# Hanbo-Cheng/DAWN-pytorch

Measured on NVIDIA H100. Metric: denoising-steps/sec (200-frame 256^2 clip), higher is better.
Workload: dtype f32

## Files before the change

### dawn_pytorch_b200/csrc/tc_common.cuh

```cuda
#pragma once
#include <cuda_fp16.h>
#include <type_traits>
#include "common.cuh"

namespace dawn {
namespace tc {

__device__ __forceinline__ uint32_t smem_u32(const void* p) { return (uint32_t)__cvta_generic_to_shared(p); }

__device__ __forceinline__ uint8_t* smem_align1024(uint8_t* base) { return base + ((1024u - (smem_u32(base) & 1023u)) & 1023u); }

template <uint32_t R>
__device__ __forceinline__ void setmaxnreg_dec() { asm volatile("setmaxnreg.dec.sync.aligned.u32 %0;" ::"n"(R)); }
template <uint32_t R>
__device__ __forceinline__ void setmaxnreg_inc() { asm volatile("setmaxnreg.inc.sync.aligned.u32 %0;" ::"n"(R)); }

template <int I, int N, class F>
__device__ __forceinline__ void static_for(F&& f) {
  if constexpr (I < N) {
    f(std::integral_constant<int, I>{});
    static_for<I + 1, N>(f);
  }
}

__device__ __forceinline__ void mbar_init(uint64_t* bar, uint32_t count) {
  asm volatile("mbarrier.init.shared::cta.b64 [%0], %1;" ::"r"(smem_u32(bar)), "r"(count));
}
__device__ __forceinline__ void mbar_arrive(uint64_t* bar) {
  asm volatile("mbarrier.arrive.shared::cta.b64 _, [%0];" ::"r"(smem_u32(bar)) : "memory");
}
__device__ __forceinline__ void mbar_arrive_relaxed(uint64_t* bar) {
  asm volatile("mbarrier.arrive.relaxed.cta.shared::cta.b64 _, [%0];" ::"r"(smem_u32(bar)) : "memory");
}
__device__ __forceinline__ void mbar_arrive_expect_tx(uint64_t* bar, uint32_t bytes) {
  asm volatile("mbarrier.arrive.expect_tx.shared::cta.b64 _, [%0], %1;" ::"r"(smem_u32(bar)), "r"(bytes) : "memory");
}
__device__ __forceinline__ void mbar_wait(uint64_t* bar, uint32_t parity) {
  asm volatile(
      "{\n\t"
      ".reg .pred p;\n\t"
      "WAIT_LOOP:\n\t"
      "mbarrier.try_wait.parity.shared::cta.b64 p, [%0], %1;\n\t"
      "@p bra WAIT_DONE;\n\t"
      "bra WAIT_LOOP;\n\t"
      "WAIT_DONE:\n\t"
      "}" ::"r"(smem_u32(bar)), "r"(parity)
      : "memory");
}
__device__ __forceinline__ void bulk_copy_g2s(void* smem_dst, const void* gsrc, uint32_t bytes, uint64_t* bar) {
  asm volatile("cp.async.bulk.shared::cluster.global.mbarrier::complete_tx::bytes [%0], [%1], %2, [%3];" ::"r"(smem_u32(smem_dst)),
               "l"(gsrc), "r"(bytes), "r"(smem_u32(bar))
               : "memory");
}
__device__ __forceinline__ void fence_proxy_async() { asm volatile("fence.proxy.async.shared::cta;" ::: "memory"); }

__device__ __forceinline__ void wgmma_fence() { asm volatile("wgmma.fence.sync.aligned;" ::: "memory"); }
__device__ __forceinline__ void wgmma_commit() { asm volatile("wgmma.commit_group.sync.aligned;" ::: "memory"); }
template <int N>
__device__ __forceinline__ void wgmma_wait() { asm volatile("wgmma.wait_group.sync.aligned %0;" ::"n"(N) : "memory"); }
__device__ __forceinline__ void wgmma_fence_acc(float (&d)[32]) {
#pragma unroll
  for (int i = 0; i < 32; ++i) asm volatile("" : "+f"(d[i])::"memory");
}
__device__ __forceinline__ void wgmma_m64n64k16(float (&d)[32], uint64_t adesc, uint64_t bdesc, uint32_t scale_d) {
  asm volatile(
      "{\n\t"
      ".reg .pred p;\n\t"
      "setp.ne.b32 p, %34, 0;\n\t"
      "wgmma.mma_async.sync.aligned.m64n64k16.f32.f16.f16 "
      "{%0, %1, %2, %3, %4, %5, %6, %7, %8, %9, %10, %11, %12, %13, %14, %15, "
      "%16, %17, %18, %19, %20, %21, %22, %23, %24, %25, %26, %27, %28, %29, %30, %31}, %32, %33, p, 1, 1, 0, 0;\n\t"
      "}"
      : "+f"(d[0]), "+f"(d[1]), "+f"(d[2]), "+f"(d[3]), "+f"(d[4]), "+f"(d[5]), "+f"(d[6]), "+f"(d[7]), "+f"(d[8]), "+f"(d[9]),
        "+f"(d[10]), "+f"(d[11]), "+f"(d[12]), "+f"(d[13]), "+f"(d[14]), "+f"(d[15]), "+f"(d[16]), "+f"(d[17]), "+f"(d[18]),
        "+f"(d[19]), "+f"(d[20]), "+f"(d[21]), "+f"(d[22]), "+f"(d[23]), "+f"(d[24]), "+f"(d[25]), "+f"(d[26]), "+f"(d[27]),
        "+f"(d[28]), "+f"(d[29]), "+f"(d[30]), "+f"(d[31])
      : "l"(adesc), "l"(bdesc), "r"(scale_d)
      : "memory");
}

__device__ __forceinline__ uint64_t make_desc(uint32_t saddr, uint32_t sbo = 1024) {
  return (uint64_t)((saddr >> 4) & 0x3FFF) | (1ull << 16) | ((uint64_t)((sbo >> 4) & 0x3FFF) << 32) | (1ull << 62);
}

constexpr int kStageLd = 68;
__device__ __forceinline__ void stage_fragment(float* stage, int r0, const float (&d)[32], bool first, int wtid) {
  const int w = wtid >> 5, l = wtid & 31;
  float* p0 = stage + (size_t)(r0 + w * 16 + (l >> 2)) * kStageLd + 2 * (l & 3);
  float* p1 = p0 + 8 * kStageLd;
#pragma unroll
  for (int j = 0; j < 8; ++j) {
    float2* a = reinterpret_cast<float2*>(p0 + 8 * j);
    float2* b = reinterpret_cast<float2*>(p1 + 8 * j);
    if (first) {
      *a = make_float2(d[4 * j], d[4 * j + 1]);
      *b = make_float2(d[4 * j + 2], d[4 * j + 3]);
    } else {
      const float2 x = *a, y = *b;
      *a = make_float2(x.x + d[4 * j], x.y + d[4 * j + 1]);
      *b = make_float2(y.x + d[4 * j + 2], y.y + d[4 * j + 3]);
    }
  }
}

__device__ __forceinline__ uint32_t swz(int r, int c) { return (uint32_t)((r >> 3) * 1024 + (r & 7) * 128 + ((c ^ (r & 7)) << 4)); }

__device__ __forceinline__ void split_f16x2(float x0, float x1, uint32_t& hi, uint32_t& lo) {
  const float h0 = __uint_as_float((__float_as_uint(x0) + 0x1000u) & 0xFFFFE000u);
  const float h1 = __uint_as_float((__float_as_uint(x1) + 0x1000u) & 0xFFFFE000u);
  const __half2 h = __floats2half2_rn(h0, h1);
  const __half2 l = __floats2half2_rn(x0 - h0, x1 - h1);
  hi = *reinterpret_cast<const uint32_t*>(&h);
  lo = *reinterpret_cast<const uint32_t*>(&l);
}

__device__ __forceinline__ void store_rows_coalesced(float* wbuf, const float (&acc)[64], float* out, size_t opix, int ldo,
                                                     int n0, bool rv, int lane) {
  float* dst[4];
#pragma unroll
  for (int k = 0; k < 4; ++k) {
    const int r = (lane >> 2) + 8 * k;
    const uint32_t lo = __shfl_sync(0xffffffffu, (uint32_t)opix, r);
    const uint32_t hi = __shfl_sync(0xffffffffu, (uint32_t)((unsigned long long)opix >> 32), r);
    const int ok = __shfl_sync(0xffffffffu, rv ? 1 : 0, r);
    const size_t px = ((size_t)hi << 32) | lo;
    dst[k] = ok ? (out + px * ldo + n0 + (lane & 3) * 4) : nullptr;
  }
#pragma unroll
  for (int pass = 0; pass < 4; ++pass) {
    __syncwarp();
#pragma unroll
    for (int j = 0; j < 4; ++j)
      *reinterpret_cast<float4*>(wbuf + lane * 20 + j * 4) =
          make_float4(acc[pass * 16 + j * 4], acc[pass * 16 + j * 4 + 1], acc[pass * 16 + j * 4 + 2], acc[pass * 16 + j * 4 + 3]);
    __syncwarp();
#pragma unroll
    for (int k = 0; k < 4; ++k) {
      const int r = (lane >> 2) + 8 * k;
      const float4 v = *reinterpret_cast<const float4*>(wbuf + r * 20 + (lane & 3) * 4);
      if (dst[k]) *reinterpret_cast<float4*>(dst[k] + pass * 16) = v;
    }
  }
}

}
}
```

### dawn_pytorch_b200/csrc/temporal_fused.cu

```cuda
#include <cuda_fp16.h>
#include <cmath>
#include <cstring>
#include <vector>
#include <algorithm>
#include "common.cuh"
#include "kernels.cuh"
#include "temporal_fused.cuh"

namespace dawn {
namespace {

constexpr int C = 64;
constexpr int X_LD = C + 8;
constexpr int W_LD = C + 8;
constexpr int K_LD = 40;
constexpr int WO_LD = 40;
constexpr int NTH = 512;
constexpr int NWARP = NTH / 32;
constexpr int W_STAGE = 2 * 96 * W_LD + 2 * 64 * WO_LD;
constexpr float LOG2E = 1.4426950408889634f;

__device__ __forceinline__ void mma16816(float (&d)[4], const uint32_t (&a)[4], uint32_t b0, uint32_t b1) {
  asm volatile(
      "mma.sync.aligned.m16n8k16.row.col.f32.f16.f16.f32 {%0,%1,%2,%3}, {%4,%5,%6,%7}, {%8,%9}, {%0,%1,%2,%3};\n"
      : "+f"(d[0]), "+f"(d[1]), "+f"(d[2]), "+f"(d[3])
      : "r"(a[0]), "r"(a[1]), "r"(a[2]), "r"(a[3]), "r"(b0), "r"(b1));
}
__device__ __forceinline__ void ldsm4(uint32_t (&r)[4], const __half* p) {
  const uint32_t addr = (uint32_t)__cvta_generic_to_shared(p);
  asm volatile("ldmatrix.sync.aligned.m8n8.x4.shared.b16 {%0,%1,%2,%3}, [%4];\n"
               : "=r"(r[0]), "=r"(r[1]), "=r"(r[2]), "=r"(r[3]) : "r"(addr));
}
__device__ __forceinline__ void ldsm4_trans(uint32_t (&r)[4], const __half* p) {
  const uint32_t addr = (uint32_t)__cvta_generic_to_shared(p);
  asm volatile("ldmatrix.sync.aligned.m8n8.x4.trans.shared.b16 {%0,%1,%2,%3}, [%4];\n"
               : "=r"(r[0]), "=r"(r[1]), "=r"(r[2]), "=r"(r[3]) : "r"(addr));
}
__device__ __forceinline__ void cp_async_16(void* dst, const void* src) {
  const uint32_t d = (uint32_t)__cvta_generic_to_shared(dst);
  asm volatile("cp.async.cg.shared.global [%0], [%1], 16;\n" :: "r"(d), "l"(src) : "memory");
}
__device__ __forceinline__ void cp_async_commit() { asm volatile("cp.async.commit_group;\n" ::: "memory"); }
__device__ __forceinline__ void cp_async_wait_all() { asm volatile("cp.async.wait_group 0;\n" ::: "memory"); }
__device__ __forceinline__ float ex2(float x) {
  float y;
  asm("ex2.approx.ftz.f32 %0, %1;\n" : "=f"(y) : "f"(x));
  return y;
}
__device__ __forceinline__ void split2h(float x0, float x1, uint32_t& hi, uint32_t& lo) {
  const float h0 = __uint_as_float(__float_as_uint(x0) & 0xFFFFE000u);
  const float h1 = __uint_as_float(__float_as_uint(x1) & 0xFFFFE000u);
  const __half2 h = __floats2half2_rn(h0, h1);
  const __half2 l = __floats2half2_rn(x0 - h0, x1 - h1);
  hi = *reinterpret_cast<const uint32_t*>(&h);
  lo = *reinterpret_cast<const uint32_t*>(&l);
}
__device__ __forceinline__ void mma3(float (&acc)[4], const uint32_t (&ah)[4], const uint32_t (&al)[4], const uint32_t (&b)[4]) {
  mma16816(acc, al, b[0], b[1]);
  mma16816(acc, ah, b[2], b[3]);
  mma16816(acc, ah, b[0], b[1]);
}

__global__ void __launch_bounds__(NTH, 1) temporal_fused_kernel(TemporalFusedArgs a) {
  extern __shared__ __align__(16) unsigned char tf_smem[];
  const int F = a.F;
  const int Fp = (F + 15) & ~15;
  const int KROWS = Fp + 32;
  const int nbuf = a.nbuf;
  __half* Xh = reinterpret_cast<__half*>(tf_smem);
  __half* Xl = Xh + Fp * X_LD;
  __half* Kh = Xl + Fp * X_LD;
  __half* Kl = Kh + KROWS * K_LD;
  __half* Vh = Kl + KROWS * K_LD;
  __half* Vl = Vh + KROWS * K_LD;
  __half* Wst = Vl + KROWS * K_LD;
  float* s_stat = reinterpret_cast<float*>(Wst + nbuf * W_STAGE);
  float* s_bias = s_stat + 2 * Fp;

  const int tid = threadIdx.x, warp = tid >> 5, lane = tid & 31;
  const int g = lane >> 2, t = lane & 3;
  const int lm = lane >> 3, lr = lane & 7;
  const int pix = blockIdx.x;
  const int band = a.band;
  const int nbias = 2 * band + 1;

  for (int i = tid; i < 8 * nbias; i += NTH) s_bias[i] = a.bias[i] * LOG2E;
  {
    const int l16 = tid & 15;
    for (int f0 = 0; f0 < Fp; f0 += NTH / 16) {
      const int f = f0 + (tid >> 4);
      float4 v = make_float4(0.f, 0.f, 0.f, 0.f);
      if (f < F) v = __ldg(reinterpret_cast<const float4*>(a.x + ((size_t)f * a.P + pix) * a.ldx) + l16);
      float s = (v.x + v.y) + (v.z + v.w);
#pragma unroll
      for (int o = 1; o < 16; o <<= 1) s += __shfl_xor_sync(0xffffffffu, s, o);
      const float mu = s * (1.0f / C);
      const float d0 = v.x - mu, d1 = v.y - mu, d2 = v.z - mu, d3 = v.w - mu;
      float ss = (d0 * d0 + d1 * d1) + (d2 * d2 + d3 * d3);
#pragma unroll
      for (int o = 1; o < 16; o <<= 1) ss += __shfl_xor_sync(0xffffffffu, ss, o);
      if (f < Fp) {
        if (l16 == 0) { s_stat[2 * f] = mu; s_stat[2 * f + 1] = 1.0f / sqrtf(ss * (1.0f / C) + 1e-5f); }
        uint32_t h0, l0, h1, l1;
        split2h(v.x, v.y, h0, l0); split2h(v.z, v.w, h1, l1);
        *reinterpret_cast<uint2*>(&Xh[f * X_LD + l16 * 4]) = make_uint2(h0, h1);
        *reinterpret_cast<uint2*>(&Xl[f * X_LD + l16 * 4]) = make_uint2(l0, l1);
      }
    }
    for (int i = tid; i < (KROWS - F) * K_LD; i += NTH) {
      Kh[F * K_LD + i] = __float2half(0.f); Kl[F * K_LD + i] = __float2half(0.f);
      Vh[F * K_LD + i] = __float2half(0.f); Vl[F * K_LD + i] = __float2half(0.f);
    }
  }

  const int ntiles = Fp >> 4;
  const int qtile = (a.q_lo >> 4) + warp;
  const bool has_q = qtile * 16 < a.q_hi;
  float y[8][4];
#pragma unroll
  for (int n = 0; n < 8; ++n)
#pragma unroll
    for (int c = 0; c < 4; ++c) y[n][c] = 0.f;

  int head_off = 0;
  const __half* Wh = Wst;
  auto stage_weights = [&](int head, __half* dst) {
    const uint4* src = reinterpret_cast<const uint4*>(a.Wqkv + (size_t)head * 2 * 96 * C);
    for (int i = tid; i < 2 * 96 * C / 8; i += NTH) {
      const int r = i / (C / 8), c8 = i - r * (C / 8);
      cp_async_16(dst + r * W_LD + c8 * 8, src + i);
    }
    const uint4* so = reinterpret_cast<const uint4*>(a.Wout + (size_t)head * 2 * 64 * 32);
    __half* od = dst + 2 * 96 * W_LD;
    for (int i = tid; i < 2 * 64 * 32 / 8; i += NTH) {
      const int r = i >> 2, c8 = i & 3;
      cp_async_16(od + r * WO_LD + c8 * 8, so + i);
    }
    cp_async_commit();
  };
  auto project = [&](int f0, int part, float (&acc)[4][4]) {
#pragma unroll
    for (int n = 0; n < 4; ++n)
#pragma unroll
      for (int c = 0; c < 4; ++c) acc[n][c] = 0.f;
#pragma unroll
    for (int ks = 0; ks < 4; ++ks) {
      uint32_t ah[4], al[4];
      const int aoff = (f0 + (lm & 1) * 8 + lr) * X_LD + ks * 16 + (lm >> 1) * 8;
      ldsm4(ah, Xh + aoff);
      ldsm4(al, Xl + aoff);
#pragma unroll
      for (int n = 0; n < 4; ++n) {
        uint32_t b[4];
        ldsm4(b, Wh + ((lm >> 1) * 96 + part * 32 + n * 8 + lr) * W_LD + ks * 16 + (lm & 1) * 8);
        mma3(acc[n], ah, al, b);
      }
    }
    const float mu0 = s_stat[2 * (f0 + g)], rs0 = s_stat[2 * (f0 + g) + 1];
    const float mu1 = s_stat[2 * (f0 + g + 8)], rs1 = s_stat[2 * (f0 + g + 8) + 1];
    const int fr0 = min(f0 + g, F - 1), fr1 = min(f0 + g + 8, F - 1);
#pragma unroll
    for (int n = 0; n < 4; ++n) {
      const float2 w = __ldg(reinterpret_cast<const float2*>(a.wsum + part * 256 + head_off + n * 8 + 2 * t));
      acc[n][0] = rs0 * (acc[n][0] * a.inv_wscale - mu0 * w.x);
      acc[n][1] = rs0 * (acc[n][1] * a.inv_wscale - mu0 * w.y);
      acc[n][2] = rs1 * (acc[n][2] * a.inv_wscale - mu1 * w.x);
      acc[n][3] = rs1 * (acc[n][3] * a.inv_wscale - mu1 * w.y);
      if (part < 2) {
        const float2 cs0 = __ldg(reinterpret_cast<const float2*>(a.rot) + (size_t)fr0 * 16 + n * 4 + t);
        const float2 cs1 = __ldg(reinterpret_cast<const float2*>(a.rot) + (size_t)fr1 * 16 + n * 4 + t);
        const float x0 = acc[n][0], x1 = acc[n][1], x2 = acc[n][2], x3 = acc[n][3];
        acc[n][0] = x0 * cs0.x - x1 * cs0.y; acc[n][1] = x1 * cs0.x + x0 * cs0.y;
        acc[n][2] = x2 * cs1.x - x3 * cs1.y; acc[n][3] = x3 * cs1.x + x2 * cs1.y;
      }
    }
  };

  if (nbuf == 2) stage_weights(0, Wst);
  for (int head = 0; head < 8; ++head) {
    if (nbuf == 2) {
      cp_async_wait_all();
      __syncthreads();
      Wh = Wst + (head & 1) * W_STAGE;
      if (head + 1 < 8) stage_weights(head + 1, Wst + ((head + 1) & 1) * W_STAGE);
    } else {
      __syncthreads();
      stage_weights(head, Wst);
      cp_async_wait_all();
      __syncthreads();
    }
    const __half* Oh = Wh + 2 * 96 * W_LD;
    head_off = head * 32;

    for (int tile = warp; tile < ntiles; tile += NWARP) {
      const int f0 = tile * 16, fr0 = f0 + g, fr1 = f0 + g + 8;
      float acc[4][4];
      project(f0, 1, acc);
#pragma unroll
      for (int n = 0; n < 4; ++n) {
        uint32_t h0, l0, h1, l1;
        split2h(acc[n][0], acc[n][1], h0, l0); split2h(acc[n][2], acc[n][3], h1, l1);
        *reinterpret_cast<uint32_t*>(&Kh[fr0 * K_LD + n * 8 + 2 * t]) = h0;
        *reinterpret_cast<uint32_t*>(&Kl[fr0 * K_LD + n * 8 + 2 * t]) = l0;
        *reinterpret_cast<uint32_t*>(&Kh[fr1 * K_LD + n * 8 + 2 * t]) = h1;
        *reinterpret_cast<uint32_t*>(&Kl[fr1 * K_LD + n * 8 + 2 * t]) = l1;
      }
      project(f0, 2, acc);
#pragma unroll
      for (int n = 0; n < 4; ++n) {
        uint32_t h0, l0, h1, l1;
        split2h(acc[n][0], acc[n][1], h0, l0); split2h(acc[n][2], acc[n][3], h1, l1);
        *reinterpret_cast<uint32_t*>(&Vh[fr0 * K_LD + n * 8 + 2 * t]) = h0;
        *reinterpret_cast<uint32_t*>(&Vl[fr0 * K_LD + n * 8 + 2 * t]) = l0;
        *reinterpret_cast<uint32_t*>(&Vh[fr1 * K_LD + n * 8 + 2 * t]) = h1;
        *reinterpret_cast<uint32_t*>(&Vl[fr1 * K_LD + n * 8 + 2 * t]) = l1;
      }
    }
    uint32_t qh[2][4], ql[2][4];
    if (has_q) {
      float acc[4][4];
      project(qtile * 16, 0, acc);
#pragma unroll
      for (int n = 0; n < 4; ++n)
#pragma unroll
        for (int c = 0; c < 4; ++c) acc[n][c] *= LOG2E;
#pragma unroll
      for (int ks = 0; ks < 2; ++ks) {
        split2h(acc[2 * ks][0], acc[2 * ks][1], qh[ks][0], ql[ks][0]);
        split2h(acc[2 * ks][2], acc[2 * ks][3], qh[ks][1], ql[ks][1]);
        split2h(acc[2 * ks + 1][0], acc[2 * ks + 1][1], qh[ks][2], ql[ks][2]);
        split2h(acc[2 * ks + 1][2], acc[2 * ks + 1][3], qh[ks][3], ql[ks][3]);
      }
    }
    __syncthreads();
    if (!has_q) continue;

    const float* bias = s_bias + head * nbias + band;
    const int i0 = qtile * 16;
    float o[4][4], mrow[2] = {-1e30f, -1e30f}, lrow[2] = {0.f, 0.f};
#pragma unroll
    for (int n = 0; n < 4; ++n)
#pragma unroll
      for (int c = 0; c < 4; ++c) o[n][c] = 0.f;
    const int kr_lo = max(0, i0 - band) & ~7, kr_hi = min(F, i0 + 16 + band);
    for (int kr0 = kr_lo; kr0 < kr_hi; kr0 += 32) {
      float s[4][4];
#pragma unroll
      for (int n = 0; n < 4; ++n)
#pragma unroll
        for (int c = 0; c < 4; ++c) s[n][c] = 0.f;
#pragma unroll
      for (int ks = 0; ks < 2; ++ks)
#pragma unroll
        for (int n = 0; n < 4; ++n) {
          uint32_t b[4];
          ldsm4(b, ((lm & 2) ? Kl : Kh) + (kr0 + n * 8 + lr) * K_LD + ks * 16 + (lm & 1) * 8);
          mma3(s[n], qh[ks], ql[ks], b);
        }
      float mnew[2] = {mrow[0], mrow[1]};
      const int rel0 = kr0 - i0 + 2 * t - g;
      const bool edge = (kr0 + 31 - i0 > band) || (kr0 - i0 - 15 < -band) || (kr0 + 32 > F);
      if (edge) {
#pragma unroll
        for (int n = 0; n < 4; ++n)
#pragma unroll
          for (int c = 0; c < 4; ++c) {
            const int rel = rel0 + n * 8 + (c & 1) - ((c & 2) ? 8 : 0);
            const bool v = ((unsigned)(rel + band) <= (unsigned)(2 * band)) && (kr0 + n * 8 + 2 * t + (c & 1) < F);
            s[n][c] = v ? s[n][c] + bias[v ? rel : 0] : -1e30f;
            mnew[c >> 1] = fmaxf(mnew[c >> 1], s[n][c]);
          }
      } else {
#pragma unroll
        for (int n = 0; n < 4; ++n)
#pragma unroll
          for (int c = 0; c < 4; ++c) {
            s[n][c] += bias[rel0 + n * 8 + (c & 1) - ((c & 2) ? 8 : 0)];
            mnew[c >> 1] = fmaxf(mnew[c >> 1], s[n][c]);
          }
      }
#pragma unroll
      for (int r = 0; r < 2; ++r) {
        mnew[r] = fmaxf(mnew[r], __shfl_xor_sync(0xffffffffu, mnew[r], 1));
        mnew[r] = fmaxf(mnew[r], __shfl_xor_sync(0xffffffffu, mnew[r], 2));
      }
      const float corr0 = ex2(mrow[0] - mnew[0]), corr1 = ex2(mrow[1] - mnew[1]);
      mrow[0] = mnew[0]; mrow[1] = mnew[1];
      float ps0 = 0.f, ps1 = 0.f;
#pragma unroll
      for (int n = 0; n < 4; ++n) {
        s[n][0] = ex2(s[n][0] - mnew[0]); s[n][1] = ex2(s[n][1] - mnew[0]);
        s[n][2] = ex2(s[n][2] - mnew[1]); s[n][3] = ex2(s[n][3] - mnew[1]);
        ps0 += s[n][0] + s[n][1]; ps1 += s[n][2] + s[n][3];
      }
      lrow[0] = lrow[0] * corr0 + ps0;
      lrow[1] = lrow[1] * corr1 + ps1;
#pragma unroll
      for (int n = 0; n < 4; ++n) { o[n][0] *= corr0; o[n][1] *= corr0; o[n][2] *= corr1; o[n][3] *= corr1; }
#pragma unroll
      for (int ks = 0; ks < 2; ++ks) {
        uint32_t ph[4], pl[4];
        split2h(s[2 * ks][0], s[2 * ks][1], ph[0], pl[0]);
        split2h(s[2 * ks][2], s[2 * ks][3], ph[1], pl[1]);
        split2h(s[2 * ks + 1][0], s[2 * ks + 1][1], ph[2], pl[2]);
        split2h(s[2 * ks + 1][2], s[2 * ks + 1][3], ph[3], pl[3]);
#pragma unroll
        for (int n = 0; n < 4; ++n) {
          uint32_t b[4];
          ldsm4_trans(b, ((lm & 2) ? Vl : Vh) + (kr0 + ks * 16 + (lm & 1) * 8 + lr) * K_LD + n * 8);
          float acc[4] = {0.f, 0.f, 0.f, 0.f};
          mma3(acc, ph, pl, b);
          o[n][0] += acc[0]; o[n][1] += acc[1]; o[n][2] += acc[2]; o[n][3] += acc[3];
        }
      }
    }
    float l0 = lrow[0], l1 = lrow[1];
    l0 += __shfl_xor_sync(0xffffffffu, l0, 1); l0 += __shfl_xor_sync(0xffffffffu, l0, 2);
    l1 += __shfl_xor_sync(0xffffffffu, l1, 1); l1 += __shfl_xor_sync(0xffffffffu, l1, 2);
    const float inv0 = 1.0f / l0, inv1 = 1.0f / l1;
    uint32_t oh[2][4], ol[2][4];
#pragma unroll
    for (int ks = 0; ks < 2; ++ks) {
      split2h(o[2 * ks][0] * inv0, o[2 * ks][1] * inv0, oh[ks][0], ol[ks][0]);
      split2h(o[2 * ks][2] * inv1, o[2 * ks][3] * inv1, oh[ks][1], ol[ks][1]);
      split2h(o[2 * ks + 1][0] * inv0, o[2 * ks + 1][1] * inv0, oh[ks][2], ol[ks][2]);
      split2h(o[2 * ks + 1][2] * inv1, o[2 * ks + 1][3] * inv1, oh[ks][3], ol[ks][3]);
    }
#pragma unroll
    for (int n = 0; n < 8; ++n) {
      float acc[4] = {0.f, 0.f, 0.f, 0.f};
#pragma unroll
      for (int ks = 0; ks < 2; ++ks) {
        uint32_t b[4];
        ldsm4(b, Oh + ((lm >> 1) * 64 + n * 8 + lr) * WO_LD + ks * 16 + (lm & 1) * 8);
        mma3(acc, oh[ks], ol[ks], b);
      }
#pragma unroll
      for (int c = 0; c < 4; ++c) y[n][c] += acc[c] * a.inv_oscale;
    }
  }

  if (has_q) {
#pragma unroll
    for (int hrow = 0; hrow < 2; ++hrow) {
      const int f = qtile * 16 + g + 8 * hrow;
      if (f < a.q_lo || f >= a.q_hi) continue;
      const size_t orow = (size_t)(f - a.q_lo) * a.P + pix;
      const float* res = a.res + orow * a.ldr;
      float* dst = a.out + orow * a.ldo;
#pragma unroll
      for (int n = 0; n < 8; ++n) {
        const float2 r = *reinterpret_cast<const float2*>(res + n * 8 + 2 * t);
        *reinterpret_cast<float2*>(dst + n * 8 + 2 * t) = make_float2(r.x + y[n][2 * hrow], r.y + y[n][2 * hrow + 1]);
      }
    }
  }
}

size_t smem_bytes(int F, int band, int nbuf) {
  const int Fp = (F + 15) & ~15, KROWS = Fp + 32;
  size_t halfs = (size_t)2 * Fp * X_LD + 4 * KROWS * K_LD + (size_t)nbuf * W_STAGE;
  return halfs * 2 + (size_t)(2 * Fp + 8 * (2 * band + 1)) * 4;
}
constexpr size_t kSmemMax = 225 * 1024;

}

bool temporal_fused_supported(int C_, int F, int band, int q_lo, int q_hi) {
  if (C_ != C || band < 1 || band > 64 || F < 1 || q_lo < 0 || q_hi > F || q_lo >= q_hi) return false;
  if (((q_hi + 15) >> 4) - (q_lo >> 4) > NWARP) return false;
  return smem_bytes(F, band, 1) <= kSmemMax;
}

int launch_temporal_fused(const TemporalFusedArgs& a_in, cudaStream_t st) {
  if (!temporal_fused_supported(C, a_in.F, a_in.band, a_in.q_lo, a_in.q_hi)) { set_last_error("temporal_fused: unsupported shape"); return -1; }
  static size_t attr_bytes = 0;
  TemporalFusedArgs a = a_in;
  a.nbuf = smem_bytes(a.F, a.band, 2) <= kSmemMax ? 2 : 1;
  const size_t smem = smem_bytes(a.F, a.band, a.nbuf);
  if (smem > attr_bytes) {
    DAWN_CUDA_OK(cudaFuncSetAttribute(temporal_fused_kernel, cudaFuncAttributeMaxDynamicSharedMemorySize, (int)smem));
    attr_bytes = smem;
  }
  temporal_fused_kernel<<<a.P, NTH, smem, st>>>(a);
  DAWN_LAUNCH_OK();
  return 0;
}

void temporal_fused_pack(const float* wqkv, const float* wout, std::vector<uint16_t>& Wq, std::vector<uint16_t>& Wo, float* inv_wscale,
                         float* inv_oscale) {
  auto pow2scale = [](const float* p, size_t n) {
    float mx = 0.f;
    for (size_t i = 0; i < n; ++i) mx = std::max(mx, std::fabs(p[i]));
    int e = 0;
    if (mx > 0.f) std::frexp(mx, &e);
    return std::ldexp(1.0f, 11 - e);
  };
  const float sq = pow2scale(wqkv, (size_t)768 * 64), so = pow2scale(wout, (size_t)64 * 256);
  *inv_wscale = 1.0f / sq; *inv_oscale = 1.0f / so;
  auto put = [](uint16_t* hi, uint16_t* lo, float v) {
    const __half h = __float2half_rn(v);
    const __half l = __float2half_rn(v - __half2float(h));
    memcpy(hi, &h, 2); memcpy(lo, &l, 2);
  };
  Wq.assign((size_t)8 * 2 * 96 * 64, 0);
  Wo.assign((size_t)8 * 2 * 64 * 32, 0);
  for (int h = 0; h < 8; ++h) {
    uint16_t* qh = Wq.data() + (size_t)h * 2 * 96 * 64; uint16_t* ql = qh + 96 * 64;
    for (int part = 0; part < 3; ++part)
      for (int r = 0; r < 32; ++r)
        for (int k = 0; k < 64; ++k)
          put(qh + (part * 32 + r) * 64 + k, ql + (part * 32 + r) * 64 + k, wqkv[(size_t)(part * 256 + h * 32 + r) * 64 + k] * sq);
    uint16_t* oh = Wo.data() + (size_t)h * 2 * 64 * 32; uint16_t* ol = oh + 64 * 32;
    for (int c = 0; c < 64; ++c)
      for (int d = 0; d < 32; ++d) put(oh + c * 32 + d, ol + c * 32 + d, wout[(size_t)c * 256 + h * 32 + d] * so);
  }
}

}
```

Baseline: 17.04.

## Use wgmma with swizzled layouts and TMA bulk weight staging in temporal attention

After: 17.39 (median of 6 runs). 1.02x the previous value.

```diff
diff --git a/dawn_pytorch_b200/csrc/tc_common.cuh b/dawn_pytorch_b200/csrc/tc_common.cuh
--- a/dawn_pytorch_b200/csrc/tc_common.cuh
+++ b/dawn_pytorch_b200/csrc/tc_common.cuh
@@ -58,9 +58,10 @@
 __device__ __forceinline__ void wgmma_commit() { asm volatile("wgmma.commit_group.sync.aligned;" ::: "memory"); }
 template <int N>
 __device__ __forceinline__ void wgmma_wait() { asm volatile("wgmma.wait_group.sync.aligned %0;" ::"n"(N) : "memory"); }
-__device__ __forceinline__ void wgmma_fence_acc(float (&d)[32]) {
+template <int N>
+__device__ __forceinline__ void wgmma_fence_acc(float (&d)[N]) {
 #pragma unroll
-  for (int i = 0; i < 32; ++i) asm volatile("" : "+f"(d[i])::"memory");
+  for (int i = 0; i < N; ++i) asm volatile("" : "+f"(d[i])::"memory");
 }
 __device__ __forceinline__ void wgmma_m64n64k16(float (&d)[32], uint64_t adesc, uint64_t bdesc, uint32_t scale_d) {
   asm volatile(
@@ -76,6 +77,32 @@
         "+f"(d[19]), "+f"(d[20]), "+f"(d[21]), "+f"(d[22]), "+f"(d[23]), "+f"(d[24]), "+f"(d[25]), "+f"(d[26]), "+f"(d[27]),
         "+f"(d[28]), "+f"(d[29]), "+f"(d[30]), "+f"(d[31])
       : "l"(adesc), "l"(bdesc), "r"(scale_d)
+      : "memory");
+}
+__device__ __forceinline__ void wgmma_m64n32k16(float (&d)[16], uint64_t adesc, uint64_t bdesc, uint32_t scale_d) {
+  asm volatile(
+      "{\n\t"
+      ".reg .pred p;\n\t"
+      "setp.ne.b32 p, %18, 0;\n\t"
+      "wgmma.mma_async.sync.aligned.m64n32k16.f32.f16.f16 "
+      "{%0, %1, %2, %3, %4, %5, %6, %7, %8, %9, %10, %11, %12, %13, %14, %15}, %16, %17, p, 1, 1, 0, 0;\n\t"
+      "}"
+      : "+f"(d[0]), "+f"(d[1]), "+f"(d[2]), "+f"(d[3]), "+f"(d[4]), "+f"(d[5]), "+f"(d[6]), "+f"(d[7]), "+f"(d[8]), "+f"(d[9]),
+        "+f"(d[10]), "+f"(d[11]), "+f"(d[12]), "+f"(d[13]), "+f"(d[14]), "+f"(d[15])
+      : "l"(adesc), "l"(bdesc), "r"(scale_d)
+      : "memory");
+}
+__device__ __forceinline__ void wgmma_m64n32k16_rs(float (&d)[16], const uint32_t (&a)[4], uint64_t bdesc, uint32_t scale_d) {
+  asm volatile(
+      "{\n\t"
+      ".reg .pred p;\n\t"
+      "setp.ne.b32 p, %21, 0;\n\t"
+      "wgmma.mma_async.sync.aligned.m64n32k16.f32.f16.f16 "
+      "{%0, %1, %2, %3, %4, %5, %6, %7, %8, %9, %10, %11, %12, %13, %14, %15}, {%16, %17, %18, %19}, %20, p, 1, 1, 0;\n\t"
+      "}"
+      : "+f"(d[0]), "+f"(d[1]), "+f"(d[2]), "+f"(d[3]), "+f"(d[4]), "+f"(d[5]), "+f"(d[6]), "+f"(d[7]), "+f"(d[8]), "+f"(d[9]),
+        "+f"(d[10]), "+f"(d[11]), "+f"(d[12]), "+f"(d[13]), "+f"(d[14]), "+f"(d[15])
+      : "r"(a[0]), "r"(a[1]), "r"(a[2]), "r"(a[3]), "l"(bdesc), "r"(scale_d)
       : "memory");
 }
 
diff --git a/dawn_pytorch_b200/csrc/temporal_fused.cu b/dawn_pytorch_b200/csrc/temporal_fused.cu
--- a/dawn_pytorch_b200/csrc/temporal_fused.cu
+++ b/dawn_pytorch_b200/csrc/temporal_fused.cu
@@ -5,20 +5,22 @@
 #include <algorithm>
 #include "common.cuh"
 #include "kernels.cuh"
+#include "tc_common.cuh"
 #include "temporal_fused.cuh"
 
 namespace dawn {
 namespace {
 
 constexpr int C = 64;
-constexpr int X_LD = C + 8;
-constexpr int W_LD = C + 8;
 constexpr int K_LD = 40;
-constexpr int WO_LD = 40;
 constexpr int NTH = 512;
 constexpr int NWARP = NTH / 32;
-constexpr int W_STAGE = 2 * 96 * W_LD + 2 * 64 * WO_LD;
 constexpr float LOG2E = 1.4426950408889634f;
+constexpr uint32_t KV_PANEL = 64 * 128;
+constexpr uint32_t Q_PANEL = 32 * 128;
+constexpr uint32_t WQKV_BYTES = 2 * KV_PANEL + 2 * Q_PANEL;
+constexpr uint32_t WOUT_BYTES = 64 * 128;
+constexpr uint32_t STAGE_BYTES = WQKV_BYTES + WOUT_BYTES;
 
 __device__ __forceinline__ void mma16816(float (&d)[4], const uint32_t (&a)[4], uint32_t b0, uint32_t b1) {
   asm volatile(
@@ -36,12 +38,6 @@
   asm volatile("ldmatrix.sync.aligned.m8n8.x4.trans.shared.b16 {%0,%1,%2,%3}, [%4];\n"
                : "=r"(r[0]), "=r"(r[1]), "=r"(r[2]), "=r"(r[3]) : "r"(addr));
 }
-__device__ __forceinline__ void cp_async_16(void* dst, const void* src) {
-  const uint32_t d = (uint32_t)__cvta_generic_to_shared(dst);
-  asm volatile("cp.async.cg.shared.global [%0], [%1], 16;\n" :: "r"(d), "l"(src) : "memory");
-}
-__device__ __forceinline__ void cp_async_commit() { asm volatile("cp.async.commit_group;\n" ::: "memory"); }
-__device__ __forceinline__ void cp_async_wait_all() { asm volatile("cp.async.wait_group 0;\n" ::: "memory"); }
 __device__ __forceinline__ float ex2(float x) {
   float y;
   asm("ex2.approx.ftz.f32 %0, %1;\n" : "=f"(y) : "f"(x));
@@ -60,34 +56,71 @@
   mma16816(acc, ah, b[2], b[3]);
   mma16816(acc, ah, b[0], b[1]);
 }
+__device__ __forceinline__ uint32_t opaque(uint32_t x) {
+  asm volatile("" : "+r"(x));
+  return x;
+}
+template <int N>
+__device__ __forceinline__ void wgmma3_k64(float (&d)[N / 2], uint32_t xh, uint32_t xl, uint32_t wh, uint32_t wl) {
+  const uint64_t ah = tc::make_desc(opaque(xh)), al = tc::make_desc(opaque(xl));
+  const uint64_t bh = tc::make_desc(opaque(wh)), bl = tc::make_desc(opaque(wl));
+  tc::wgmma_fence();
+#pragma unroll
+  for (int ks = 0; ks < 4; ++ks) {
+    const uint64_t o = (uint64_t)(ks * 2);
+    if constexpr (N == 64) {
+      tc::wgmma_m64n64k16(d, al + o, bh + o, ks > 0 ? 1u : 0u);
+      tc::wgmma_m64n64k16(d, ah + o, bl + o, 1u);
+      tc::wgmma_m64n64k16(d, ah + o, bh + o, 1u);
+    } else {
+      tc::wgmma_m64n32k16(d, al + o, bh + o, ks > 0 ? 1u : 0u);
+      tc::wgmma_m64n32k16(d, ah + o, bl + o, 1u);
+      tc::wgmma_m64n32k16(d, ah + o, bh + o, 1u);
+    }
+  }
+  tc::wgmma_commit();
+  tc::wgmma_wait<0>();
+  tc::wgmma_fence_acc(d);
+}
 
 __global__ void __launch_bounds__(NTH, 1) temporal_fused_kernel(TemporalFusedArgs a) {
-  extern __shared__ __align__(16) unsigned char tf_smem[];
+  extern __shared__ __align__(1024) uint8_t tf_smem[];
   const int F = a.F;
   const int Fp = (F + 15) & ~15;
+  const int XR = Fp + 48;
   const int KROWS = Fp + 32;
   const int nbuf = a.nbuf;
-  __half* Xh = reinterpret_cast<__half*>(tf_smem);
-  __half* Xl = Xh + Fp * X_LD;
-  __half* Kh = Xl + Fp * X_LD;
+  uint8_t* Wst = tc::smem_align1024(tf_smem);
+  uint8_t* Xh = Wst + nbuf * STAGE_BYTES;
+  uint8_t* Xl = Xh + XR * 128;
+  __half* Kh = reinterpret_cast<__half*>(Xl + XR * 128);
   __half* Kl = Kh + KROWS * K_LD;
   __half* Vh = Kl + KROWS * K_LD;
   __half* Vl = Vh + KROWS * K_LD;
-  __half* Wst = Vl + KROWS * K_LD;
-  float* s_stat = reinterpret_cast<float*>(Wst + nbuf * W_STAGE);
-  float* s_bias = s_stat + 2 * Fp;
-
-  const int tid = threadIdx.x, warp = tid >> 5, lane = tid & 31;
+  float* s_stat = reinterpret_cast<float*>(Vl + KROWS * K_LD);
+  float* s_bias = s_stat + 2 * XR;
+  const int band = a.band;
+  const int nbias = 2 * band + 1;
+  float* s_wsum = s_bias + 8 * nbias;
+  uint64_t* wfull = reinterpret_cast<uint64_t*>(s_wsum + 2 * 96);
+
+  const int tid = threadIdx.x, warp = tid >> 5, lane = tid & 31, wg = warp >> 2;
   const int g = lane >> 2, t = lane & 3;
   const int lm = lane >> 3, lr = lane & 7;
   const int pix = blockIdx.x;
-  const int band = a.band;
-  const int nbias = 2 * band + 1;
-
+
+  if (tid == 0) {
+    for (int s = 0; s < nbuf; ++s) tc::mbar_init(&wfull[s], 1);
+    asm volatile("fence.mbarrier_init.release.cluster;" ::: "memory");
+  }
   for (int i = tid; i < 8 * nbias; i += NTH) s_bias[i] = a.bias[i] * LOG2E;
+  auto stage_wsum = [&](int head) {
+    if (tid < 96) s_wsum[(head & 1) * 96 + tid] = __ldg(a.wsum + (tid >> 5) * 256 + head * 32 + (tid & 31));
+  };
+  stage_wsum(0);
   {
     const int l16 = tid & 15;
-    for (int f0 = 0; f0 < Fp; f0 += NTH / 16) {
+    for (int f0 = 0; f0 < XR; f0 += NTH / 16) {
       const int f = f0 + (tid >> 4);
       float4 v = make_float4(0.f, 0.f, 0.f, 0.f);
       if (f < F) v = __ldg(reinterpret_cast<const float4*>(a.x + ((size_t)f * a.P + pix) * a.ldx) + l16);
@@ -99,131 +132,116 @@
       float ss = (d0 * d0 + d1 * d1) + (d2 * d2 + d3 * d3);
 #pragma unroll
       for (int o = 1; o < 16; o <<= 1) ss += __shfl_xor_sync(0xffffffffu, ss, o);
-      if (f < Fp) {
+      if (f < XR) {
         if (l16 == 0) { s_stat[2 * f] = mu; s_stat[2 * f + 1] = 1.0f / sqrtf(ss * (1.0f / C) + 1e-5f); }
         uint32_t h0, l0, h1, l1;
         split2h(v.x, v.y, h0, l0); split2h(v.z, v.w, h1, l1);
-        *reinterpret_cast<uint2*>(&Xh[f * X_LD + l16 * 4]) = make_uint2(h0, h1);
-        *reinterpret_cast<uint2*>(&Xl[f * X_LD + l16 * 4]) = make_uint2(l0, l1);
-      }
-    }
+        const uint32_t off = f * 128 + ((((l16 >> 1) ^ (f & 7)) << 4) | ((l16 & 1) << 3));
+        *reinterpret_cast<uint2*>(Xh + off) = make_uint2(h0, h1);
+        *reinterpret_cast<uint2*>(Xl + off) = make_uint2(l0, l1);
+      }
+    }
+    tc::fence_proxy_async();
     for (int i = tid; i < (KROWS - F) * K_LD; i += NTH) {
       Kh[F * K_LD + i] = __float2half(0.f); Kl[F * K_LD + i] = __float2half(0.f);
       Vh[F * K_LD + i] = __float2half(0.f); Vl[F * K_LD + i] = __float2half(0.f);
     }
   }
 
-  const int ntiles = Fp >> 4;
   const int qtile = (a.q_lo >> 4) + warp;
   const bool has_q = qtile * 16 < a.q_hi;
+  const int q0 = 16 * (a.q_lo >> 4) + 64 * wg;
+  const bool wg_q = q0 < a.q_hi;
   float y[8][4];
 #pragma unroll
   for (int n = 0; n < 8; ++n)
 #pragma unroll
     for (int c = 0; c < 4; ++c) y[n][c] = 0.f;
 
-  int head_off = 0;
-  const __half* Wh = Wst;
-  auto stage_weights = [&](int head, __half* dst) {
-    const uint4* src = reinterpret_cast<const uint4*>(a.Wqkv + (size_t)head * 2 * 96 * C);
-    for (int i = tid; i < 2 * 96 * C / 8; i += NTH) {
-      const int r = i / (C / 8), c8 = i - r * (C / 8);
-      cp_async_16(dst + r * W_LD + c8 * 8, src + i);
-    }
-    const uint4* so = reinterpret_cast<const uint4*>(a.Wout + (size_t)head * 2 * 64 * 32);
-    __half* od = dst + 2 * 96 * W_LD;
-    for (int i = tid; i < 2 * 64 * 32 / 8; i += NTH) {
-      const int r = i >> 2, c8 = i & 3;
-      cp_async_16(od + r * WO_LD + c8 * 8, so + i);
-    }
-    cp_async_commit();
-  };
-  auto project = [&](int f0, int part, float (&acc)[4][4]) {
-#pragma unroll
-    for (int n = 0; n < 4; ++n)
-#pragma unroll
-      for (int c = 0; c < 4; ++c) acc[n][c] = 0.f;
-#pragma unroll
-    for (int ks = 0; ks < 4; ++ks) {
-      uint32_t ah[4], al[4];
-      const int aoff = (f0 + (lm & 1) * 8 + lr) * X_LD + ks * 16 + (lm >> 1) * 8;
-      ldsm4(ah, Xh + aoff);
-      ldsm4(al, Xl + aoff);
-#pragma unroll
-      for (int n = 0; n < 4; ++n) {
-        uint32_t b[4];
-        ldsm4(b, Wh + ((lm >> 1) * 96 + part * 32 + n * 8 + lr) * W_LD + ks * 16 + (lm & 1) * 8);
-        mma3(acc[n], ah, al, b);
-      }
-    }
+  const float2* rot = reinterpret_cast<const float2*>(a.rot);
+  auto prefetch_rot = [&](int f) {
+    asm volatile("prefetch.global.L1 [%0];" ::"l"(rot + (size_t)min(f, F - 1) * 16));
+    asm volatile("prefetch.global.L1 [%0];" ::"l"(rot + (size_t)min(f + 8, F - 1) * 16));
+  };
+  auto fold = [&](float (&v)[4], int f0, int part, const float* wsum, int n) {
     const float mu0 = s_stat[2 * (f0 + g)], rs0 = s_stat[2 * (f0 + g) + 1];
     const float mu1 = s_stat[2 * (f0 + g + 8)], rs1 = s_stat[2 * (f0 + g + 8) + 1];
-    const int fr0 = min(f0 + g, F - 1), fr1 = min(f0 + g + 8, F - 1);
-#pragma unroll
-    for (int n = 0; n < 4; ++n) {
-      const float2 w = __ldg(reinterpret_cast<const float2*>(a.wsum + part * 256 + head_off + n * 8 + 2 * t));
-      acc[n][0] = rs0 * (acc[n][0] * a.inv_wscale - mu0 * w.x);
-      acc[n][1] = rs0 * (acc[n][1] * a.inv_wscale - mu0 * w.y);
-      acc[n][2] = rs1 * (acc[n][2] * a.inv_wscale - mu1 * w.x);
-      acc[n][3] = rs1 * (acc[n][3] * a.inv_wscale - mu1 * w.y);
-      if (part < 2) {
-        const float2 cs0 = __ldg(reinterpret_cast<const float2*>(a.rot) + (size_t)fr0 * 16 + n * 4 + t);
-        const float2 cs1 = __ldg(reinterpret_cast<const float2*>(a.rot) + (size_t)fr1 * 16 + n * 4 + t);
-        const float x0 = acc[n][0], x1 = acc[n][1], x2 = acc[n][2], x3 = acc[n][3];
-        acc[n][0] = x0 * cs0.x - x1 * cs0.y; acc[n][1] = x1 * cs0.x + x0 * cs0.y;
-        acc[n][2] = x2 * cs1.x - x3 * cs1.y; acc[n][3] = x3 * cs1.x + x2 * cs1.y;
-      }
-    }
-  };
-
-  if (nbuf == 2) stage_weights(0, Wst);
+    const float2 w = *reinterpret_cast<const float2*>(wsum + part * 32 + n * 8 + 2 * t);
+    v[0] = rs0 * (v[0] * a.inv_wscale - mu0 * w.x);
+    v[1] = rs0 * (v[1] * a.inv_wscale - mu0 * w.y);
+    v[2] = rs1 * (v[2] * a.inv_wscale - mu1 * w.x);
+    v[3] = rs1 * (v[3] * a.inv_wscale - mu1 * w.y);
+    if (part < 2) {
+      const int fr0 = min(f0 + g, F - 1), fr1 = min(f0 + g + 8, F - 1);
+      const float2 cs0 = __ldg(rot + (size_t)fr0 * 16 + n * 4 + t);
+      const float2 cs1 = __ldg(rot + (size_t)fr1 * 16 + n * 4 + t);
+      const float x0 = v[0], x1 = v[1], x2 = v[2], x3 = v[3];
+      v[0] = x0 * cs0.x - x1 * cs0.y; v[1] = x1 * cs0.x + x0 * cs0.y;
+      v[2] = x2 * cs1.x - x3 * cs1.y; v[3] = x3 * cs1.x + x2 * cs1.y;
+    }
+  };
+  auto stage_weights = [&](int head, int s) {
+    tc::mbar_arrive_expect_tx(&wfull[s], STAGE_BYTES);
+    tc::bulk_copy_g2s(Wst + s * STAGE_BYTES, a.Wqkv + (size_t)head * (WQKV_BYTES / 2), WQKV_BYTES, &wfull[s]);
+    tc::bulk_copy_g2s(Wst + s * STAGE_BYTES + WQKV_BYTES, a.Wout + (size_t)head * (WOUT_BYTES / 2), WOUT_BYTES, &wfull[s]);
+  };
+
+  const uint32_t xh = tc::smem_u32(Xh), xl = tc::smem_u32(Xl);
+  if (nbuf == 2 && tid == 0) stage_weights(0, 0);
   for (int head = 0; head < 8; ++head) {
-    if (nbuf == 2) {
-      cp_async_wait_all();
-      __syncthreads();
-      Wh = Wst + (head & 1) * W_STAGE;
-      if (head + 1 < 8) stage_weights(head + 1, Wst + ((head + 1) & 1) * W_STAGE);
-    } else {
-      __syncthreads();
-      stage_weights(head, Wst);
-      cp_async_wait_all();
-      __syncthreads();
-    }
-    const __half* Oh = Wh + 2 * 96 * W_LD;
-    head_off = head * 32;
-
-    for (int tile = warp; tile < ntiles; tile += NWARP) {
-      const int f0 = tile * 16, fr0 = f0 + g, fr1 = f0 + g + 8;
+    __syncthreads();
+    if (tid == 0) {
+      if (nbuf == 1) stage_weights(head, 0);
+      else if (head + 1 < 8) stage_weights(head + 1, (head + 1) & 1);
+    }
+    if (head + 1 < 8) stage_wsum(head + 1);
+    const int s = nbuf == 2 ? (head & 1) : 0;
+    tc::mbar_wait(&wfull[s], nbuf == 2 ? (head >> 1) & 1 : head & 1);
+    const uint32_t w = tc::smem_u32(Wst + s * STAGE_BYTES);
+    const float* wsum = s_wsum + (head & 1) * 96;
+
+    for (int tile = wg; tile * 64 < F; tile += 4) {
+      const int f0 = tile * 64 + 16 * (warp & 3), fr0 = f0 + g, fr1 = f0 + g + 8;
+      prefetch_rot(fr0);
+      float d[32];
+      wgmma3_k64<64>(d, xh + tile * 64 * 128, xl + tile * 64 * 128, w, w + KV_PANEL);
+#pragma unroll
+      for (int part = 1; part < 3; ++part) {
+        __half* ph = part == 1 ? Kh : Vh;
+        __half* pl = part == 1 ? Kl : Vl;
+#pragma unroll
+        for (int n = 0; n < 4; ++n) {
+          const int j = 4 * (part - 1) + n;
+          float v[4] = {d[4 * j], d[4 * j + 1], d[4 * j + 2], d[4 * j + 3]};
+          fold(v, f0, part, wsum, n);
+          uint32_t h0, l0, h1, l1;
+          split2h(v[0], v[1], h0, l0); split2h(v[2], v[3], h1, l1);
+          const int col = n * 8 + 2 * t;
+          if (fr0 < F) {
+            *reinterpret_cast<uint32_t*>(&ph[fr0 * K_LD + col]) = h0;
+            *reinterpret_cast<uint32_t*>(&pl[fr0 * K_LD + col]) = l0;
+          }
+          if (fr1 < F) {
+            *reinterpret_cast<uint32_t*>(&ph[fr1 * K_LD + col]) = h1;
+            *reinterpret_cast<uint32_t*>(&pl[fr1 * K_LD + col]) = l1;
+          }
+        }
+      }
+    }
+    uint32_t qh[2][4], ql[2][4];
+    if (wg_q) {
+      prefetch_rot(qtile * 16 + g);
+      float d[16];
+      wgmma3_k64<32>(d, xh + q0 * 128, xl + q0 * 128, w + 2 * KV_PANEL, w + 2 * KV_PANEL + Q_PANEL);
       float acc[4][4];
-      project(f0, 1, acc);
 #pragma unroll
       for (int n = 0; n < 4; ++n) {
-        uint32_t h0, l0, h1, l1;
-        split2h(acc[n][0], acc[n][1], h0, l0); split2h(acc[n][2], acc[n][3], h1, l1);
-        *reinterpret_cast<uint32_t*>(&Kh[fr0 * K_LD + n * 8 + 2 * t]) = h0;
-        *reinterpret_cast<uint32_t*>(&Kl[fr0 * K_LD + n * 8 + 2 * t]) = l0;
-        *reinterpret_cast<uint32_t*>(&Kh[fr1 * K_LD + n * 8 + 2 * t]) = h1;
-        *reinterpret_cast<uint32_t*>(&Kl[fr1 * K_LD + n * 8 + 2 * t]) = l1;
-      }
-      project(f0, 2, acc);
-#pragma unroll
-      for (int n = 0; n < 4; ++n) {
-        uint32_t h0, l0, h1, l1;
-        split2h(acc[n][0], acc[n][1], h0, l0); split2h(acc[n][2], acc[n][3], h1, l1);
-        *reinterpret_cast<uint32_t*>(&Vh[fr0 * K_LD + n * 8 + 2 * t]) = h0;
-        *reinterpret_cast<uint32_t*>(&Vl[fr0 * K_LD + n * 8 + 2 * t]) = l0;
-        *reinterpret_cast<uint32_t*>(&Vh[fr1 * K_LD + n * 8 + 2 * t]) = h1;
-        *reinterpret_cast<uint32_t*>(&Vl[fr1 * K_LD + n * 8 + 2 * t]) = l1;
-      }
-    }
-    uint32_t qh[2][4], ql[2][4];
-    if (has_q) {
-      float acc[4][4];
-      project(qtile * 16, 0, acc);
-#pragma unroll
-      for (int n = 0; n < 4; ++n)
+#pragma unroll
+        for (int c = 0; c < 4; ++c) acc[n][c] = d[4 * n + c];
+        fold(acc[n], qtile * 16, 0, wsum, n);
 #pragma unroll
         for (int c = 0; c < 4; ++c) acc[n][c] *= LOG2E;
+      }
 #pragma unroll
       for (int ks = 0; ks < 2; ++ks) {
         split2h(acc[2 * ks][0], acc[2 * ks][1], qh[ks][0], ql[ks][0]);
@@ -233,110 +251,125 @@
       }
     }
     __syncthreads();
-    if (!has_q) continue;
-
-    const float* bias = s_bias + head * nbias + band;
-    const int i0 = qtile * 16;
-    float o[4][4], mrow[2] = {-1e30f, -1e30f}, lrow[2] = {0.f, 0.f};
-#pragma unroll
-    for (int n = 0; n < 4; ++n)
-#pragma unroll
-      for (int c = 0; c < 4; ++c) o[n][c] = 0.f;
-    const int kr_lo = max(0, i0 - band) & ~7, kr_hi = min(F, i0 + 16 + band);
-    for (int kr0 = kr_lo; kr0 < kr_hi; kr0 += 32) {
-      float s[4][4];
+    if (!wg_q) continue;
+
+    uint32_t oh[2][4], ol[2][4];
+#pragma unroll
+    for (int ks = 0; ks < 2; ++ks)
+#pragma unroll
+      for (int c = 0; c < 4; ++c) oh[ks][c] = ol[ks][c] = 0u;
+    if (has_q) {
+      const float* bias = s_bias + head * nbias + band;
+      const int i0 = qtile * 16;
+      float o[4][4], mrow[2] = {-1e30f, -1e30f}, lrow[2] = {0.f, 0.f};
 #pragma unroll
       for (int n = 0; n < 4; ++n)
 #pragma unroll
-        for (int c = 0; c < 4; ++c) s[n][c] = 0.f;
-#pragma unroll
-      for (int ks = 0; ks < 2; ++ks)
+        for (int c = 0; c < 4; ++c) o[n][c] = 0.f;
+      const int kr_lo = max(0, i0 - band) & ~7, kr_hi = min(F, i0 + 16 + band);
+      for (int kr0 = kr_lo; kr0 < kr_hi; kr0 += 32) {
+        float s[4][4];
+#pragma unroll
+        for (int n = 0; n < 4; ++n)
+#pragma unroll
+          for (int c = 0; c < 4; ++c) s[n][c] = 0.f;
+#pragma unroll
+        for (int ks = 0; ks < 2; ++ks)
+#pragma unroll
+          for (int n = 0; n < 4; ++n) {
+            uint32_t b[4];
+            ldsm4(b, ((lm & 2) ? Kl : Kh) + (kr0 + n * 8 + lr) * K_LD + ks * 16 + (lm & 1) * 8);
+            mma3(s[n], qh[ks], ql[ks], b);
+          }
+        float mnew[2] = {mrow[0], mrow[1]};
+        const int rel0 = kr0 - i0 + 2 * t - g;
+        const bool edge = (kr0 + 31 - i0 > band) || (kr0 - i0 - 15 < -band) || (kr0 + 32 > F);
+        if (edge) {
+#pragma unroll
+          for (int n = 0; n < 4; ++n)
+#pragma unroll
+            for (int c = 0; c < 4; ++c) {
+              const int rel = rel0 + n * 8 + (c & 1) - ((c & 2) ? 8 : 0);
+              const bool v = ((unsigned)(rel + band) <= (unsigned)(2 * band)) && (kr0 + n * 8 + 2 * t + (c & 1) < F);
+              s[n][c] = v ? s[n][c] + bias[v ? rel : 0] : -1e30f;
+              mnew[c >> 1] = fmaxf(mnew[c >> 1], s[n][c]);
+            }
+        } else {
+#pragma unroll
+          for (int n = 0; n < 4; ++n)
+#pragma unroll
+            for (int c = 0; c < 4; ++c) {
+              s[n][c] += bias[rel0 + n * 8 + (c & 1) - ((c & 2) ? 8 : 0)];
+              mnew[c >> 1] = fmaxf(mnew[c >> 1], s[n][c]);
+            }
+        }
+#pragma unroll
+        for (int r = 0; r < 2; ++r) {
+          mnew[r] = fmaxf(mnew[r], __shfl_xor_sync(0xffffffffu, mnew[r], 1));
+          mnew[r] = fmaxf(mnew[r], __shfl_xor_sync(0xffffffffu, mnew[r], 2));
+        }
+        const float corr0 = ex2(mrow[0] - mnew[0]), corr1 = ex2(mrow[1] - mnew[1]);
+        mrow[0] = mnew[0]; mrow[1] = mnew[1];
+        float ps0 = 0.f, ps1 = 0.f;
 #pragma unroll
         for (int n = 0; n < 4; ++n) {
-          uint32_t b[4];
-          ldsm4(b, ((lm & 2) ? Kl : Kh) + (kr0 + n * 8 + lr) * K_LD + ks * 16 + (lm & 1) * 8);
-          mma3(s[n], qh[ks], ql[ks], b);
+          s[n][0] = ex2(s[n][0] - mnew[0]); s[n][1] = ex2(s[n][1] - mnew[0]);
+          s[n][2] = ex2(s[n][2] - mnew[1]); s[n][3] = ex2(s[n][3] - mnew[1]);
+          ps0 += s[n][0] + s[n][1]; ps1 += s[n][2] + s[n][3];
         }
-      float mnew[2] = {mrow[0], mrow[1]};
-      const int rel0 = kr0 - i0 + 2 * t - g;
-      const bool edge = (kr0 + 31 - i0 > band) || (kr0 - i0 - 15 < -band) || (kr0 + 32 > F);
-      if (edge) {
-#pragma unroll
-        for (int n = 0; n < 4; ++n)
-#pragma unroll
-          for (int c = 0; c < 4; ++c) {
-            const int rel = rel0 + n * 8 + (c & 1) - ((c & 2) ? 8 : 0);
-            const bool v = ((unsigned)(rel + band) <= (unsigned)(2 * band)) && (kr0 + n * 8 + 2 * t + (c & 1) < F);
-            s[n][c] = v ? s[n][c] + bias[v ? rel : 0] : -1e30f;
-            mnew[c >> 1] = fmaxf(mnew[c >> 1], s[n][c]);
+        lrow[0] = lrow[0] * corr0 + ps0;
+        lrow[1] = lrow[1] * corr1 + ps1;
+#pragma unroll
+        for (int n = 0; n < 4; ++n) { o[n][0] *= corr0; o[n][1] *= corr0; o[n][2] *= corr1; o[n][3] *= corr1; }
+#pragma unroll
+        for (int ks = 0; ks < 2; ++ks) {
+          uint32_t ph[4], pl[4];
+          split2h(s[2 * ks][0], s[2 * ks][1], ph[0], pl[0]);
+          split2h(s[2 * ks][2], s[2 * ks][3], ph[1], pl[1]);
+          split2h(s[2 * ks + 1][0], s[2 * ks + 1][1], ph[2], pl[2]);
+          split2h(s[2 * ks + 1][2], s[2 * ks + 1][3], ph[3], pl[3]);
+#pragma unroll
+          for (int n = 0; n < 4; ++n) {
+            uint32_t b[4];
+            ldsm4_trans(b, ((lm & 2) ? Vl : Vh) + (kr0 + ks * 16 + (lm & 1) * 8 + lr) * K_LD + n * 8);
+            float acc[4] = {0.f, 0.f, 0.f, 0.f};
+            mma3(acc, ph, pl, b);
+            o[n][0] += acc[0]; o[n][1] += acc[1]; o[n][2] += acc[2]; o[n][3] += acc[3];
           }
-      } else {
-#pragma unroll
-        for (int n = 0; n < 4; ++n)
-#pragma unroll
-          for (int c = 0; c < 4; ++c) {
-            s[n][c] += bias[rel0 + n * 8 + (c & 1) - ((c & 2) ? 8 : 0)];
-            mnew[c >> 1] = fmaxf(mnew[c >> 1], s[n][c]);
-          }
-      }
-#pragma unroll
-      for (int r = 0; r < 2; ++r) {
-        mnew[r] = fmaxf(mnew[r], __shfl_xor_sync(0xffffffffu, mnew[r], 1));
-        mnew[r] = fmaxf(mnew[r], __shfl_xor_sync(0xffffffffu, mnew[r], 2));
-      }
-      const float corr0 = ex2(mrow[0] - mnew[0]), corr1 = ex2(mrow[1] - mnew[1]);
-      mrow[0] = mnew[0]; mrow[1] = mnew[1];
-      float ps0 = 0.f, ps1 = 0.f;
-#pragma unroll
-      for (int n = 0; n < 4; ++n) {
-        s[n][0] = ex2(s[n][0] - mnew[0]); s[n][1] = ex2(s[n][1] - mnew[0]);
-        s[n][2] = ex2(s[n][2] - mnew[1]); s[n][3] = ex2(s[n][3] - mnew[1]);
-        ps0 += s[n][0] + s[n][1]; ps1 += s[n][2] + s[n][3];
-      }
-      lrow[0] = lrow[0] * corr0 + ps0;
-      lrow[1] = lrow[1] * corr1 + ps1;
-#pragma unroll
-      for (int n = 0; n < 4; ++n) { o[n][0] *= corr0; o[n][1] *= corr0; o[n][2] *= corr1; o[n][3] *= corr1; }
+        }
+      }
+      float l0 = lrow[0], l1 = lrow[1];
+      l0 += __shfl_xor_sync(0xffffffffu, l0, 1); l0 += __shfl_xor_sync(0xffffffffu, l0, 2);
+      l1 += __shfl_xor_sync(0xffffffffu, l1, 1); l1 += __shfl_xor_sync(0xffffffffu, l1, 2);
+      const float inv0 = 1.0f / l0, inv1 = 1.0f / l1;
 #pragma unroll
       for (int ks = 0; ks < 2; ++ks) {
-        uint32_t ph[4], pl[4];
-        split2h(s[2 * ks][0], s[2 * ks][1], ph[0], pl[0]);
-        split2h(s[2 * ks][2], s[2 * ks][3], ph[1], pl[1]);
-        split2h(s[2 * ks + 1][0], s[2 * ks + 1][1], ph[2], pl[2]);
-        split2h(s[2 * ks + 1][2], s[2 * ks + 1][3], ph[3], pl[3]);
-#pragma unroll
-        for (int n = 0; n < 4; ++n) {
-          uint32_t b[4];
-          ldsm4_trans(b, ((lm & 2) ? Vl : Vh) + (kr0 + ks * 16 + (lm & 1) * 8 + lr) * K_LD + n * 8);
-          float acc[4] = {0.f, 0.f, 0.f, 0.f};
-          mma3(acc, ph, pl, b);
-          o[n][0] += acc[0]; o[n][1] += acc[1]; o[n][2] += acc[2]; o[n][3] += acc[3];
-        }
-      }
-    }
-    float l0 = lrow[0], l1 = lrow[1];
-    l0 += __shfl_xor_sync(0xffffffffu, l0, 1); l0 += __shfl_xor_sync(0xffffffffu, l0, 2);
-    l1 += __shfl_xor_sync(0xffffffffu, l1, 1); l1 += __shfl_xor_sync(0xffffffffu, l1, 2);
-    const float inv0 = 1.0f / l0, inv1 = 1.0f / l1;
-    uint32_t oh[2][4], ol[2][4];
-#pragma unroll
-    for (int ks = 0; ks < 2; ++ks) {
-      split2h(o[2 * ks][0] * inv0, o[2 * ks][1] * inv0, oh[ks][0], ol[ks][0]);
-      split2h(o[2 * ks][2] * inv1, o[2 * ks][3] * inv1, oh[ks][1], ol[ks][1]);
-      split2h(o[2 * ks + 1][0] * inv0, o[2 * ks + 1][1] * inv0, oh[ks][2], ol[ks][2]);
-      split2h(o[2 * ks + 1][2] * inv1, o[2 * ks + 1][3] * inv1, oh[ks][3], ol[ks][3]);
-    }
-#pragma unroll
-    for (int n = 0; n < 8; ++n) {
-      float acc[4] = {0.f, 0.f, 0.f, 0.f};
+        split2h(o[2 * ks][0] * inv0, o[2 * ks][1] * inv0, oh[ks][0], ol[ks][0]);
+        split2h(o[2 * ks][2] * inv1, o[2 * ks][3] * inv1, oh[ks][1], ol[ks][1]);
+        split2h(o[2 * ks + 1][0] * inv0, o[2 * ks + 1][1] * inv0, oh[ks][2], ol[ks][2]);
+        split2h(o[2 * ks + 1][2] * inv1, o[2 * ks + 1][3] * inv1, oh[ks][3], ol[ks][3]);
+      }
+    }
+#pragma unroll
+    for (int half = 0; half < 2; ++half) {
+      float d[16];
+      const uint64_t bo = tc::make_desc(opaque(w + WQKV_BYTES + half * 32 * 128));
+      constexpr uint64_t LO = 64 / 16;
+      tc::wgmma_fence();
 #pragma unroll
       for (int ks = 0; ks < 2; ++ks) {
-        uint32_t b[4];
-        ldsm4(b, Oh + ((lm >> 1) * 64 + n * 8 + lr) * WO_LD + ks * 16 + (lm & 1) * 8);
-        mma3(acc, oh[ks], ol[ks], b);
-      }
-#pragma unroll
-      for (int c = 0; c < 4; ++c) y[n][c] += acc[c] * a.inv_oscale;
+        const uint64_t o = (uint64_t)(ks * 2);
+        tc::wgmma_m64n32k16_rs(d, ol[ks], bo + o, ks > 0 ? 1u : 0u);
+        tc::wgmma_m64n32k16_rs(d, oh[ks], bo + LO + o, 1u);
+        tc::wgmma_m64n32k16_rs(d, oh[ks], bo + o, 1u);
+      }
+      tc::wgmma_commit();
+      tc::wgmma_wait<0>();
+      tc::wgmma_fence_acc(d);
+#pragma unroll
+      for (int n = 0; n < 4; ++n)
+#pragma unroll
+        for (int c = 0; c < 4; ++c) y[4 * half + n][c] += d[4 * n + c] * a.inv_oscale;
     }
   }
 
@@ -358,9 +391,9 @@
 }
 
 size_t smem_bytes(int F, int band, int nbuf) {
-  const int Fp = (F + 15) & ~15, KROWS = Fp + 32;
-  size_t halfs = (size_t)2 * Fp * X_LD + 4 * KROWS * K_LD + (size_t)nbuf * W_STAGE;
-  return halfs * 2 + (size_t)(2 * Fp + 8 * (2 * band + 1)) * 4;
+  const int Fp = (F + 15) & ~15, XR = Fp + 48, KROWS = Fp + 32;
+  return 1024 + (size_t)nbuf * STAGE_BYTES + (size_t)2 * XR * 128 + (size_t)4 * KROWS * K_LD * 2 +
+         (size_t)(2 * XR + 8 * (2 * band + 1) + 2 * 96) * 4 + 2 * sizeof(uint64_t);
 }
 constexpr size_t kSmemMax = 225 * 1024;
 
@@ -398,23 +431,30 @@
   };
   const float sq = pow2scale(wqkv, (size_t)768 * 64), so = pow2scale(wout, (size_t)64 * 256);
   *inv_wscale = 1.0f / sq; *inv_oscale = 1.0f / so;
+  auto at = [](int r, int k) { return (size_t)(r * 64 + (((k >> 3) ^ (r & 7)) << 3) + (k & 7)); };
   auto put = [](uint16_t* hi, uint16_t* lo, float v) {
     const __half h = __float2half_rn(v);
     const __half l = __float2half_rn(v - __half2float(h));
     memcpy(hi, &h, 2); memcpy(lo, &l, 2);
   };
-  Wq.assign((size_t)8 * 2 * 96 * 64, 0);
-  Wo.assign((size_t)8 * 2 * 64 * 32, 0);
+  constexpr size_t KVH = KV_PANEL / 2, QH = Q_PANEL / 2;
+  Wq.assign((size_t)8 * WQKV_BYTES / 2, 0);
+  Wo.assign((size_t)8 * WOUT_BYTES / 2, 0);
   for (int h = 0; h < 8; ++h) {
-    uint16_t* qh = Wq.data() + (size_t)h * 2 * 96 * 64; uint16_t* ql = qh + 96 * 64;
-    for (int part = 0; part < 3; ++part)
-      for (int r = 0; r < 32; ++r)
-        for (int k = 0; k < 64; ++k)
-          put(qh + (part * 32 + r) * 64 + k, ql + (part * 32 + r) * 64 + k, wqkv[(size_t)(part * 256 + h * 32 + r) * 64 + k] * sq);
-    uint16_t* oh = Wo.data() + (size_t)h * 2 * 64 * 32; uint16_t* ol = oh + 64 * 32;
+    uint16_t* kvh = Wq.data() + (size_t)h * WQKV_BYTES / 2;
+    uint16_t* kvl = kvh + KVH;
+    uint16_t* qh = kvl + KVH;
+    uint16_t* ql = qh + QH;
+    for (int r = 0; r < 32; ++r)
+      for (int k = 0; k < 64; ++k) {
+        put(qh + at(r, k), ql + at(r, k), wqkv[(size_t)(h * 32 + r) * 64 + k] * sq);
+        put(kvh + at(r, k), kvl + at(r, k), wqkv[(size_t)(256 + h * 32 + r) * 64 + k] * sq);
+        put(kvh + at(32 + r, k), kvl + at(32 + r, k), wqkv[(size_t)(512 + h * 32 + r) * 64 + k] * sq);
+      }
+    uint16_t* o = Wo.data() + (size_t)h * WOUT_BYTES / 2;
     for (int c = 0; c < 64; ++c)
-      for (int d = 0; d < 32; ++d) put(oh + c * 32 + d, ol + c * 32 + d, wout[(size_t)c * 256 + h * 32 + d] * so);
-  }
-}
-
-}
+      for (int d = 0; d < 32; ++d) put(o + at(c, d), o + at(c, 32 + d), wout[(size_t)c * 256 + h * 32 + d] * so);
+  }
+}
+
+}
```
